# MiniMax-AI/VTP

Measured on AMD Instinct MI355X. Metric: images/sec/node VTP-B f16d64 256x256 train step, higher is better.
Workload: dtype bf16

## Files before the change

vtp_amd/csrc/gemm4w_tn.hip:

```cpp
#include "gemm_common.h"
#include "gemm_group.h"
#include "diag.h"
#include "gemm4w_tn_ktile.inc"

namespace vtp {

namespace {
constexpr int W4T_KT = 65536;
constexpr int W4T_RING = 2 * W4T_KT;
constexpr int W4T_LDS = W4T_RING + 32768;
}

__device__ __forceinline__ void w4t_glds16(const char* sbase, unsigned voff, unsigned lds_dst) {
  unsigned keep;
  asm volatile("s_mov_b32 %0, m0\n\ts_mov_b32 m0, %3\n\ts_nop 0\n\tglobal_load_lds_dwordx4 %1, %2\n\ts_mov_b32 m0, %0"
               : "=&s"(keep)
               : "v"(voff), "s"(sbase), "s"(lds_dst)
               : "memory");
}

__device__ __forceinline__ int w4t_uni(long v) { return __builtin_amdgcn_readfirstlane((int)v); }
template <class T>
__device__ __forceinline__ T* w4t_uni(T* v) {
  const unsigned long long u = (unsigned long long)v;
  const unsigned lo = __builtin_amdgcn_readfirstlane((unsigned)u), hi = __builtin_amdgcn_readfirstlane((unsigned)(u >> 32));
  return (T*)(((unsigned long long)hi << 32) | lo);
}

struct W4TStage {
  const char *mata, *matb, *zb;
  unsigned stepa, stepb, da[2], db[2];
};

__device__ __forceinline__ void w4t_kloop(bool csum, f32x16 (&acc)[4][4], float (&cs)[4], const unsigned (&aE)[2], const unsigned (&aO)[2],
                                          const unsigned (&bE)[2], const unsigned (&bO)[2], unsigned& pea, unsigned& peb, unsigned zoff,
                                          const W4TStage& st, int& kra, int& krb, unsigned nk2) {
  unsigned vt, sm, cnt = nk2;
  unsigned long long sb;
  const unsigned ones = 0x3F803F80u;
  const unsigned docs = __builtin_amdgcn_readfirstlane(csum ? 1u : 0u);
  asm volatile(W4T_TILE_ASM_BOTH
               : W4T_TILE_ACC, [cs0] "+v"(cs[0]), [cs1] "+v"(cs[1]), [cs2] "+v"(cs[2]), [cs3] "+v"(cs[3]), [pea] "+v"(pea), [peb] "+v"(peb),
                 [vt] "=&v"(vt), [kra] "+s"(kra), [krb] "+s"(krb), [cnt] "+s"(cnt), [sm] "=&s"(sm), [sb] "=&s"(sb)
               : [aE0] "v"(aE[0]), [aO0] "v"(aO[0]), [bE0] "v"(bE[0]), [bO0] "v"(bO[0]), [aE1] "v"(aE[1]), [aO1] "v"(aO[1]), [bE1] "v"(bE[1]),
                 [bO1] "v"(bO[1]), [zoff] "v"(zoff), [mata] "s"(st.mata), [matb] "s"(st.matb), [zb] "s"(st.zb), [stepa] "s"(st.stepa),
                 [stepb] "s"(st.stepb), [ones] "s"(ones), [docs] "s"(docs), [da0] "s"(st.da[0]), [da1] "s"(st.da[1]), [db0] "s"(st.db[0]),
                 [db1] "s"(st.db[1])
               : "memory", "scc", "vcc", W4T_TILE_CLOBBERS);
}

__device__ __forceinline__ void w4t_segment(const GroupArgs& ga, int tile, int kbeg, int kcount, int nparts, int part) {
  extern __shared__ __attribute__((aligned(16))) char smem[];
  const int tid = threadIdx.x;
  auto stamp = [&](int which) {
    if (__builtin_expect(ga.timing != nullptr, 0) && tid == 0) diag_stamp(ga.timing, (size_t)blockIdx.x * 8 + which);
  };
  if (__builtin_expect(ga.timing != nullptr, 0) && tid == 0) {
    ga.timing[(size_t)blockIdx.x * 8 + 5] = (unsigned long long)tile;
    ga.timing[(size_t)blockIdx.x * 8 + 6] = (unsigned long long)part;
    unsigned xcc;
    asm volatile("s_getreg_b32 %0, hwreg(HW_REG_XCC_ID)" : "=s"(xcc));
    ga.timing[(size_t)blockIdx.x * 8 + 7] = (unsigned long long)(xcc & 15);
  }
  stamp(0);
  const int lane = tid & 63;
  const int wave = __builtin_amdgcn_readfirstlane(tid >> 6);
  const int wr = wave >> 1, wc = wave & 1;
  const int hi = lane >> 5;

  int g = 0;
  for (int i = 1; i < ga.nprob; ++i)
    if ((int)ga.probs[i].tile0 <= tile) g = i;
  const GroupProblem& pr = ga.probs[g];
  GemmArgs p{};
  p.A = w4t_uni(pr.A); p.B = w4t_uni(pr.B); p.C = w4t_uni(pr.C); p.resid = w4t_uni(pr.accumulate) ? (const float*)p.C : nullptr;
  p.colsum = w4t_uni(pr.colsum);
  p.M = w4t_uni(pr.M); p.N = w4t_uni(pr.N); p.K = w4t_uni(pr.K) > 0 ? w4t_uni(pr.K) : ga.K; p.lda = w4t_uni(pr.lda); p.ldb = w4t_uni(pr.ldb); p.ldc = w4t_uni(pr.ldc);
  p.c_grp = w4t_uni(pr.c_grp); p.c_pre = w4t_uni(pr.c_pre); p.k_split = ga.k_split; p.alpha = 1.f;
  p.xcd_swizzle = 2;
  const int lt = tile - w4t_uni(pr.tile0), tiles_n = (p.N + 255) >> 8;
  const int n0 = (lt % tiles_n) << 8, m0 = (lt / tiles_n) << 8;
  kcount = max(0, min(kcount, p.K - kbeg));
  const unsigned nk2 = (unsigned)max(1, (kcount + 127) >> 7);

  const int krow = lane >> 3, chunk = (lane & 7) ^ (4 * ((krow >> 1) & 1));
  const int cola = min(m0 + wave * 64 + chunk * 8, p.M - 8), colb = min(n0 + wave * 64 + chunk * 8, p.N - 8);
  unsigned pea = (unsigned)(((size_t)(kbeg + krow) * p.lda + cola) * 2), peb = (unsigned)(((size_t)(kbeg + krow) * p.ldb + colb) * 2);
  const unsigned zoff = (lane & 3) * 16;
  W4TStage st;
  st.mata = (const char*)p.A;
  st.matb = (const char*)p.B;
  st.zb = (const char*)g_zero_block;
  st.stepa = (unsigned)(8 * p.lda * 2);
  st.stepb = (unsigned)(8 * p.ldb * 2);
#pragma unroll
  for (int sl = 0; sl < 2; ++sl) {
    st.da[sl] = (unsigned)(size_t)smem + sl * W4T_KT + wave * 8192;
    st.db[sl] = st.da[sl] + 32768;
  }
#pragma unroll
  for (int kt = 0; kt < 2; ++kt)
#pragma unroll
    for (int i = 0; i < 8; ++i) {
      const bool valid = kt * 64 + 8 * i < kcount;
      w4t_glds16(valid ? st.mata : st.zb, valid ? pea : zoff, st.da[kt] + i * 1024);
      w4t_glds16(valid ? st.matb : st.zb, valid ? peb : zoff, st.db[kt] + i * 1024);
      pea += st.stepa;
      peb += st.stepb;
    }
  int kra = kcount - 128, krb = kcount - 128;

  unsigned aE[2], aO[2], bE[2], bO[2];
  {
    const int t_li = lane & 15, t_rq = t_li >> 2;
    const int cq = ((lane >> 4) & 1) * 2 + ((t_li & 3) >> 1), sz = 4 * ((t_rq >> 1) & 1);
    const unsigned rowb = (unsigned)((hi * 8 + t_rq) * 128 + (t_li & 1) * 8);
    const unsigned lb0 = rowb + (unsigned)(((0 + cq) ^ sz) << 4), lb1 = rowb + (unsigned)(((4 + cq) ^ sz) << 4);
#pragma unroll
    for (int sl = 0; sl < 2; ++sl) {
      const unsigned ba = (unsigned)(size_t)smem + sl * W4T_KT + (wr * 2) * 8192, bb = (unsigned)(size_t)smem + sl * W4T_KT + (4 + wc * 2) * 8192;
      aE[sl] = ba + lb0;
      aO[sl] = ba + lb1;
      bE[sl] = bb + lb0;
      bO[sl] = bb + lb1;
    }
  }
  f32x16 acc[4][4];
#pragma unroll
  for (int i = 0; i < 4; ++i)
#pragma unroll
    for (int j = 0; j < 4; ++j)
#pragma unroll
      for (int e = 0; e < 16; ++e) acc[i][j][e] = 0.f;
  float cs[4] = {0.f, 0.f, 0.f, 0.f};
  const bool do_csum = p.colsum != nullptr && n0 == 0;

  asm volatile("s_waitcnt vmcnt(0)" ::: "memory");
  __builtin_amdgcn_s_barrier();
  __builtin_amdgcn_sched_barrier(0);
  stamp(1);
  w4t_kloop(do_csum, acc, cs, aE, aO, bE, bO, pea, peb, zoff, st, kra, krb, nk2);
  asm volatile("s_nop 15\n\ts_nop 15\n\ts_nop 7\n\ts_waitcnt vmcnt(0)" ::: "memory");
  stamp(2);

  if (do_csum && wc == 0) {
#pragma unroll
    for (int j = 0; j < 4; ++j) {
      const float v = cs[j] + __shfl_xor(cs[j], 32, 64);
      const int m = m0 + wr * 128 + j * 32 + (lane & 31);
      if (hi == 0 && m < p.M) unsafeAtomicAdd(p.colsum + remap_row(m, p.c_grp, p.c_pre), v);
    }
  }
  if (nparts > 1) {
    typedef __attribute__((ext_vector_type(4))) unsigned int u32x4_t;
    const f32x4* mine = (const f32x4*)ga.part + (((size_t)tile * ga.splits + part) * 4 + wave) * 4096;
    const auto rsrc = __builtin_amdgcn_make_buffer_rsrc((void*)mine, 0, 4096 * 16, 0x00020000);
#pragma unroll
    for (int u = 0; u < 64; ++u) {
      f32x4 v;
#pragma unroll
      for (int e = 0; e < 4; ++e) v[e] = acc[u >> 4][(u >> 2) & 3][4 * (u & 3) + e];
      __builtin_amdgcn_raw_buffer_store_b128((u32x4_t)v, rsrc, lane * 16 + u * 1024, 0,  16);
    }
    asm volatile("s_waitcnt vmcnt(0)" ::: "memory");
    __syncthreads();
    int* flag = (int*)(smem + W4T_LDS - 16);
    if (tid == 0) {
      const int t = __hip_atomic_fetch_add(ga.ticket + tile, 1, __ATOMIC_RELAXED, __HIP_MEMORY_SCOPE_AGENT);
      const int last = t == nparts - 1;
      if (last) {
        __builtin_amdgcn_fence(__ATOMIC_ACQUIRE, "agent");
        __hip_atomic_store(ga.ticket + tile, 0, __ATOMIC_RELAXED, __HIP_MEMORY_SCOPE_AGENT);
      }
      *flag = last;
    }
    __syncthreads();
    stamp(3);
    if (*flag == 0) return;
    for (int z = 0; z < nparts; ++z) {
      if (z == part) continue;
      const f32x4* other = (const f32x4*)ga.part + (((size_t)tile * ga.splits + z) * 4 + wave) * 4096 + lane;
      constexpr int NLD = 16;
#pragma unroll
      for (int gq = 0; gq < 64 / NLD; ++gq) {
        f32x4 v[NLD];
#pragma unroll
        for (int t = 0; t < NLD; ++t) v[t] = other[(gq * NLD + t) * 64];
#pragma unroll
        for (int t = 0; t < NLD; ++t) {
          const int u = gq * NLD + t;
#pragma unroll
          for (int e = 0; e < 4; ++e) acc[u >> 4][(u >> 2) & 3][4 * (u & 3) + e] += v[t][e];
        }
        asm volatile("" ::: "memory");
      }
    }
  }
  char* reg = smem + W4T_RING + wave * 8192;
  gemm_epilogue<EPI_F32, false, 128, 64, 4096, 0>(p, *(f32x16(*)[2][4]) & acc[0], reg, m0, n0, wr, wc * 2, lane, 0, nullptr);
  gemm_epilogue<EPI_F32, false, 128, 64, 4096, 0>(p, *(f32x16(*)[2][4]) & acc[2], reg, m0, n0, wr, wc * 2 + 1, lane, 0, nullptr);
  stamp(4);
}


__global__ __launch_bounds__(256, 1) void gemm4w_grouped_tn_items_kernel(const GroupArgs ga) {
  const int c = xcd_chunk_start(blockIdx.x, gridDim.x) + ((int)blockIdx.x >> 3);
  const GroupItem& it = ga.items[c];
  w4t_segment(ga, w4t_uni(it.tile), w4t_uni(it.kbeg), w4t_uni(it.kcount), w4t_uni(it.nparts), w4t_uni(it.part));
}

int launch_gemm4w_grouped_tn_items(const GroupArgs& ga, int nitems, hipStream_t s) {
  static bool attr_set = false;
  if (!attr_set) {
    (void)hipFuncSetAttribute((const void*)gemm4w_grouped_tn_items_kernel, hipFuncAttributeMaxDynamicSharedMemorySize, W4T_LDS);
    attr_set = true;
  }
  hipLaunchKernelGGL(gemm4w_grouped_tn_items_kernel, dim3(nitems), dim3(256), W4T_LDS, s, ga);
  return check_launch("gemm4w_grouped_tn_items");
}

}
```

vtp_amd/csrc/gemm8p.hip:

```cpp
#include "gemm_common.h"
#include "gemm_group.h"
#include "diag.h"
#include <cstdlib>
#include <type_traits>

namespace vtp {

namespace {
constexpr int P8_SLOT = 16384;
constexpr int P8_RING = 8 * P8_SLOT;
constexpr int P8_REGION = 4096;
constexpr int P8_LDS = P8_RING + 8 * P8_REGION;
}

__device__ __forceinline__ void p8_wait_vm_halftiles(int n) {
  if (n >= 4) asm volatile("s_waitcnt vmcnt(8)" ::: "memory");
  else if (n == 3) asm volatile("s_waitcnt vmcnt(6)" ::: "memory");
  else if (n == 2) asm volatile("s_waitcnt vmcnt(4)" ::: "memory");
  else if (n == 1) asm volatile("s_waitcnt vmcnt(2)" ::: "memory");
  else asm volatile("s_waitcnt vmcnt(0)" ::: "memory");
}

__device__ __forceinline__ void p8_glds16(const char* sbase, unsigned voff, unsigned lds_dst) {
  unsigned keep;
// ... 562 lines not shown
    return launch_persistent<kern, gemm8p_dyn_kernel<EPI, VAR, XMODE>>(a, ntiles, 1, 512, P8_LDS, 4, s, "gemm8p_nt");
  else
    return launch_persistent<kern, nullptr>(a, ntiles, 1, 512, P8_LDS, 4, s, TRANS ? "gemm8p_tn" : "gemm8p_nt");
}

bool gemm8p_fits(const GemmArgs& a, bool trans) {
  const size_t lim = (size_t)1 << 32;
  if (trans) return (size_t)a.K * a.lda * 2 < lim && (size_t)a.K * a.ldb * 2 < lim;
  size_t rows_a = a.M;
  if (a.a_grp > 0) rows_a += ((size_t)a.M / a.a_grp + 1) * a.a_pre;
  return rows_a * a.lda * 2 < lim && (size_t)a.N * a.ldb * 2 < lim;
}

int launch_gemm8p_nt(const GemmArgs& a, int epi, int splits, hipStream_t s) {
  switch (epi) {
    case EPI_BF16:
      if (a.rope_pos) return launch8p<EPI_BF16, false, 0, 1>(a, splits, s);
      if (a.swiglu_pre) return launch8p<EPI_BF16, false, 0, 2>(a, splits, s);
      return launch8p<EPI_BF16, false, 0, 0>(a, splits, s);
    case EPI_F32: return launch8p<EPI_F32, false>(a, splits, s);
    case EPI_SWIGLU: return launch8p<EPI_SWIGLU, false>(a, splits, s);
    case EPI_GELU: return launch8p<EPI_GELU, false>(a, splits, s);
    case EPI_F32_ATOMIC: return launch8p<EPI_F32_ATOMIC, false>(a, splits, s);
    case EPI_F32_SLAB: return launch8p<EPI_F32_SLAB, false>(a, splits, s);
    default: set_error("gemm8p: unsupported epilogue %d", epi); return VTP_ERR_ARG;
  }
}

int launch_gemm8p_nt_fp8(const GemmArgs& a, int epi, hipStream_t s) {
  switch (epi) {
    case EPI_BF16: return a.rope_pos ? launch8p<EPI_BF16, false, 8, 1>(a, 1, s) : launch8p<EPI_BF16, false, 8, 0>(a, 1, s);
    case EPI_F32: return launch8p<EPI_F32, false, 8>(a, 1, s);
    case EPI_SWIGLU: return launch8p<EPI_SWIGLU, false, 8>(a, 1, s);
    default: set_error("gemm8p fp8: unsupported epilogue %d", epi); return VTP_ERR_ARG;
  }
}

int launch_gemm8p_tn(const GemmArgs& a, int epi, int splits, hipStream_t s) {
  if (epi == EPI_F32) return launch8p<EPI_F32, true>(a, 1, s);
  if (epi == EPI_F32_ATOMIC) return launch8p<EPI_F32_ATOMIC, true>(a, splits, s);
  return launch8p<EPI_F32_SLAB, true>(a, splits, s);
}

}

namespace vtp {
int launch_gemm4w_grouped_tn_items(const GroupArgs& ga, int nitems, hipStream_t s);
}
static int launch_gemm8p_grouped_tn(const void* probs, int nprob, int ntiles, int K, int splits, void* part, void* ticket,
                                    const int* k_rows, void* stream) {
  using namespace vtp;
  if (k_rows) { splits = 1; part = ticket = nullptr; }
  GroupArgs ga{};
  ga.probs = (const GroupProblem*)probs; ga.part = (float*)part; ga.ticket = (int*)ticket;
  ga.nprob = nprob; ga.ntiles = ntiles; ga.K = K;
  ga.k_split = ((K + splits - 1) / splits + 63) / 64 * 64;
  ga.splits = (K + ga.k_split - 1) / ga.k_split;
  ga.timing = g_p8_timing;
  ga.k_rows = k_rows;
  auto* kern = k_rows ? gemm8p_grouped_tn_limit_kernel : gemm8p_grouped_tn_kernel;
  static bool attr_set[2] = {false, false};
  if (!attr_set[k_rows != nullptr]) {
    hipFuncSetAttribute((const void*)kern, hipFuncAttributeMaxDynamicSharedMemorySize, P8_LDS);
    attr_set[k_rows != nullptr] = true;
  }
  hipLaunchKernelGGL(kern, dim3(ntiles * ga.splits), dim3(512), P8_LDS, (hipStream_t)stream, ga);
  return check_launch("gemm8p_grouped_tn");
}
extern "C" int vtp_gemm_tn_grouped(const void* probs, int nprob, int ntiles, int K, int splits, void* part, void* ticket,
                                   void* stream) {
  VTP_REQUIRE(probs && nprob >= 1 && nprob <= 8, "vtp_gemm_tn_grouped: 1..8 problems");
  VTP_REQUIRE(ntiles >= 1 && K >= 1 && splits >= 1, "vtp_gemm_tn_grouped: bad shape (ntiles %d, K %d, splits %d)", ntiles, K, splits);
  VTP_REQUIRE(splits == 1 || (part && ticket), "vtp_gemm_tn_grouped: split-K needs the partial-sum and ticket buffers");
  return launch_gemm8p_grouped_tn(probs, nprob, ntiles, K, splits, part, ticket, nullptr, stream);
}
extern "C" int vtp_gemm_tn_grouped_limit(const void* probs, int nprob, int ntiles, int K, const int* k_rows, void* stream) {
  VTP_REQUIRE(probs && k_rows && nprob >= 1 && nprob <= 8, "vtp_gemm_tn_grouped_limit: 1..8 problems and a row count");
  VTP_REQUIRE(ntiles >= 1 && K >= 1, "vtp_gemm_tn_grouped_limit: bad shape (ntiles %d, K %d)", ntiles, K);
  return launch_gemm8p_grouped_tn(probs, nprob, ntiles, K, 1, nullptr, nullptr, k_rows, stream);
}
extern "C" int vtp_gemm_tn_grouped_items(const void* probs, int nprob, int ntiles, int K, const void* items, int nitems, int slots,
                                         void* part, void* ticket, void* stream) {
  using namespace vtp;
  VTP_REQUIRE(probs && nprob >= 1 && nprob <= 8, "vtp_gemm_tn_grouped_items: 1..8 problems");
  VTP_REQUIRE(items && nitems >= ntiles && ntiles >= 1 && K >= 8 && K % 8 == 0 && slots >= 1,
              "vtp_gemm_tn_grouped_items: bad shape (ntiles %d, nitems %d, K %d, slots %d)", ntiles, nitems, K, slots);
  VTP_REQUIRE(slots == 1 || (part && ticket), "vtp_gemm_tn_grouped_items: split tiles need the partial-sum and ticket buffers");
  GroupArgs ga{};
  ga.probs = (const GroupProblem*)probs; ga.part = (float*)part; ga.ticket = (int*)ticket;
  ga.nprob = nprob; ga.ntiles = ntiles; ga.K = K; ga.k_split = K; ga.splits = slots;
  ga.timing = g_p8_timing;
  ga.items = (const GroupItem*)items;
  return launch_gemm4w_grouped_tn_items(ga, nitems, (hipStream_t)stream);
}

extern "C" int vtp_set_gemm_dynamic(int on) {
  vtp::g_dyn_mode = on ? 1 : 0;
  return VTP_OK;
}

extern "C" int vtp_gemm_debug(void* timing, int grid_limit, int delay_ticks) {
  const bool off = timing == nullptr && grid_limit == 0 && delay_ticks == 0;
  if (!off && !vtp::diag_allowed("vtp_gemm_debug")) return VTP_ERR_ARG;
  if (delay_ticks < 0 || grid_limit < 0) {
    vtp::set_error("vtp_gemm_debug: negative grid limit / delay");
    return VTP_ERR_ARG;
  }
  vtp::g_p8_timing = (unsigned long long*)timing;
  vtp::g_p8_grid = grid_limit;
  vtp::g_p8_delay = delay_ticks;
  return VTP_OK;
}
```

vtp_amd/engine.py:

```python
from __future__ import annotations

import math
import os
from typing import Dict, List, NamedTuple, Optional, Tuple

import torch

from . import ops
from .ops import EPI_BF16, EPI_F32, EPI_F32_SLAB, EPI_GELU, EPI_SWIGLU


class Lin:
    __slots__ = ("N", "K", "w", "wT", "bias", "gw", "gb", "w32", "wTs")


class SwiGLULin:
    __slots__ = ("H", "K", "w12", "w12T", "b12", "gw1", "gb1")


def _flat_order(names: List[str]) -> List[str]:
    out, seen = [], set()
    for n in names:
        if n in seen:
            continue
# ... 767 lines not shown
        xmid = ws.get("xmid", (M, D), F32)
        hid = ws.get("hid", (M, H), BF)
        rope_plan = self._rope_plan(ws, segs, prefix_tokens, M)
        rope_arg = None if rope_plan is None else (rope_plan[0], rope_plan[1], rope_plan[2], 2 * D)
        rows = self._attn_rows(segs)
        for i, b in enumerate(self.blocks):
            w8, al, sc = f["w"][i], f["alpha"][i], f["act_scale"][i]
            xout = ws.get(f"xout{i & 1}", (M, D), F32)
            ops.norm_fwd_e4m3(x, b.n1w, b.n1b, a8, sc[0:1], None, M, D, self.eps, self.kind)
            if b.qn_w is not None:
                qkv_pre = ws.get("f8.qkv_pre", (M, 3 * D), BF)
                ops.gemm_nt_fp8(a8, w8[0], qkv_pre, M=M, N=3 * D, K=D, alpha=al[0], bias=b.qkv.bias, epi=EPI_BF16)
                ops.qk_norm_fwd(qkv_pre, b.qn_w, b.kn_w, qkv, ws.get("f8.qinv", (M, 2 * heads), F32), M, D)
            else:
                ops.gemm_nt_fp8(a8, w8[0], qkv, M=M, N=3 * D, K=D, alpha=al[0], bias=b.qkv.bias, epi=EPI_BF16, rope=rope_arg)
            self._attention(qkv, o, lse, rows, i, prefix_tokens, rope_arg is None)
            ops.quantize_e4m3(o, a8, sc[1:2])
            ops.gemm_nt_fp8(a8, w8[1], xmid, M=M, N=D, K=D, alpha=al[1], bias=b.proj.bias, resid=x, epi=EPI_F32)
            ops.norm_fwd_e4m3(xmid, b.n2w, b.n2b, a8, sc[2:3], None, M, D, self.eps, self.kind)
            ops.gemm_nt_fp8(a8, w8[2], hid, M=M, N=2 * H, K=D, alpha=al[2], bias=b.w12.b12, epi=EPI_SWIGLU)
            ops.quantize_e4m3(hid, a8, sc[3:4])
            ops.gemm_nt_fp8(a8, w8[3], xout, M=M, N=D, K=H, alpha=al[3], bias=b.w3.bias, resid=xmid, epi=EPI_F32)
            x = xout
        return x

    def fp32_check(self, what: str):
        if self.qk_norm:
            raise NotImplementedError(f"fp32 forward ({what}): QK normalisation (use_qk_norm) is not implemented in fp32")
        if self.D % 8 or self.H % 8 or self.D != self.heads * 64:
            raise NotImplementedError(f"fp32 forward ({what}): needs D, H multiples of 8 and head dimension 64 (D={self.D} H={self.H} heads={self.heads})")

    def _forward_fp32(self, ws: Workspace, x, segs, prefix_tokens: int, M: int, keep: bool = False):
        self.fp32_check(self.style)
        D, H, heads = self.D, self.H, self.heads
        xn, st = ws.get("f32.xn", (M, D), F32), ws.get("f32.st", (M, 2), F32)
        qkv, o = ws.get("f32.qkv", (M, 3 * D), F32), ws.get("f32.o", (M, D), F32)
        xmid, hid = ws.get("f32.xmid", (M, D), F32), ws.get("f32.hid", (M, H), F32)
        rows = self._attn_rows(segs)
        for i, b in enumerate(self.blocks):
            xout = ws.get(f"f32.{i}.xout" if keep else f"f32.xout{i & 1}", (M, D), F32)
            ops.norm_fwd_f32(x, b.n1w, b.n1b, xn, st, M, D, self.eps, self.kind)
            ops.gemm_nt_f32(xn, b.qkv.w32, qkv, M=M, N=3 * D, K=D, bias=b.qkv.bias)
            for r0, Bs, Ns, rp in rows:
                q_s, o_s = qkv[r0:r0 + Bs * Ns], o[r0:r0 + Bs * Ns]
                if rp is not None:
                    rs, rc = rope_at(rp, i)
                    ops.rope_qk_f32(q_s, rs, rc, Bs, Ns, heads, prefix_tokens)
                ops.attn_fwd_f32(q_s, q_s[:, D:], q_s[:, 2 * D:], o_s, Bs, Ns, heads, Ns * 3 * D, 3 * D, Ns * D, D, ATTN_SCALE, self.causal)
            ops.gemm_nt_f32(o, b.proj.w32, xmid, M=M, N=D, K=D, bias=b.proj.bias, gamma=b.ls1, resid=x, epi=ops.F32_RESID)
            ops.norm_fwd_f32(xmid, b.n2w, b.n2b, xn, st, M, D, self.eps, self.kind)
            if self.swiglu:
                ops.gemm_nt_f32(xn, b.w1_32, hid, M=M, N=H, K=D, w2=b.w2_32, bias=b.b1_32, bias2=b.b2_32, epi=ops.F32_SWIGLU)
            else:
                ops.gemm_nt_f32(xn, b.fc.w32, hid, M=M, N=H, K=D, bias=b.fc.bias,
                                epi=ops.F32_QUICK_GELU if self.quick_gelu else ops.F32_GELU)
            ops.gemm_nt_f32(hid, b.w3.w32, xout, M=M, N=D, K=H, bias=b.w3.bias, gamma=b.ls2, resid=xmid, epi=ops.F32_RESID)
            x = xout
        return x

    def w3_colsum_target(self, i: int):
        b = self.blocks[i]
        return b.w3.gb if (b.ls2 is None and self.drop_plan is None) else None

    def backward(self, ws: Workspace, dy, dy_b, segs, prefix_tokens: int, saved=None, dy_colsum_done: bool = False,
                 hold_last: bool = False, extra_last=None):
        D, H = self.D, self.H
        M = sum(b * n for b, n, _ in segs)
        saved = self.last_saved if saved is None else saved
        tail_Mc = saved[-1].o_c.shape[0] if saved and saved[-1].row_map is not None else None
        drop = self.drop_plan is not None
        if drop:
            csegs, Mb = self._drop_segs(segs)
            rows, scales, bt = list(self._rows(csegs)), self.drop_plan["scales"], "b.d."
            gdy, gdy_b = ws.get(bt + "gdy", (Mb, D), F32), ws.get(bt + "gdy_b", (Mb, D), BF)
            dxc = ws.get(bt + "dxc", (Mb, D), F32)
        else:
            Mb, rows, bt = M, self._attn_rows(segs), "b."
            dmid = ws.get("b.dmid", (M, D), F32)
        grouped = not drop and M >= 256 and all(b.ls1 is None and b.ls2 is None for b in self.blocks) \
            and ops.wgrad_group_fits(M, max(3 * D, 2 * H if self.swiglu else H)) and D % 8 == 0 and H % 8 == 0
        vl = self.varlen
        if vl is not None and not (grouped and tail_Mc is None and len(segs) == 1 and not extra_last):
            raise RuntimeError("Stack.backward: packed captions need the grouped weight gradients of one plain segment (varlen_ok)")
        par = (lambda i: f".{i & 1}") if grouped else (lambda i: "")
        groups = ws.__dict__.setdefault("_wgrad_groups", {})
        scratch = self.__dict__.setdefault("_wgrad_scratch", {})
        pending = None

        def launch_pending():
            if pending is None:
                return
            if OVERLAP.enabled:
                OVERLAP.fork()
                side, grp = OVERLAP.side, pending[1]

                def issue():
                    with torch.cuda.stream(side):
                        grp.launch()
                OVERLAP.defer(issue)
            else:
                pending[1].launch()

        for i in range(self.depth - 1, -1, -1):
            b, s = self.blocks[i], saved[i]
            t = f"{i}.d." if drop else f"{i}."
            dpre = ws.get(bt + "dx12" + par(i), (Mb, 2 * H if self.swiglu else H), BF)
            dqkv = ws.get(bt + "dqkv" + par(i), (Mb, 3 * D), BF)
            if drop:
                self._gather(dy, segs, csegs, i, 1, gdy, gdy_b, scales)
                self._ffn_bwd(ws, i, s, gdy, gdy_b, dxc, None, Mb, bt, dpre, fused=False)
                self._scatter(dxc, dy, segs, csegs, i, 1, 1.0, accumulate=False)
                self._gather(dy, segs, csegs, i, 0, gdy, gdy_b, scales)
                self._attn_bwd(ws, t, i, s, gdy, gdy_b, dxc, None, Mb, bt, dqkv, rows, prefix_tokens)
                self._scatter(dxc, dy, segs, csegs, i, 0, 1.0, accumulate=False)
                OVERLAP.join()
                yield ("block", i)
                continue
            dxo = ws.get(f"b.dx{i & 1}", (M, D), F32)
            dxo_b = ws.get(f"b.dx_b{i & 1}", (M, D), BF)
            Mf = tail_Mc if (tail_Mc is not None and i == self.depth - 1) else M
            if Mf != M:
                dpre = ws.get(bt + "dx12" + par(i), (Mf, 2 * H if self.swiglu else H), BF)
            dmid = ws.get("b.dmid", (Mf, D), F32)
            dmid_b = ws.get("b.dmid_b" + par(i), (Mf, D), BF)
            probs = [] if grouped else None
            if grouped:
                launch_pending()
            self._ffn_bwd(ws, i, s, dy, dy_b, dmid, dmid_b, Mf, bt, dpre, fused=self.swiglu and b.ls2 is None,
                          bias_done=dy_colsum_done if i == self.depth - 1 else self.w3_colsum_target(i) is not None, probs=probs,
                          dx_colsum=b.proj.gb if b.ls1 is None else None)
            self._attn_bwd(ws, t, i, s, dmid, dmid_b, dxo, dxo_b, M, bt, dqkv, rows, prefix_tokens, bias_done=b.proj.gb is not None,
                           probs=probs, join=grouped, dx_colsum=self.w3_colsum_target(i - 1) if i > 0 else None)
            dy, dy_b = dxo, dxo_b
            if not grouped:
                OVERLAP.join()
                yield ("block", i)
                continue
            extra = [dict(pr, dy=dy_b) for pr in extra_last] if (i == 0 and hold_last and extra_last) else []
            gkey = (i, bool(self.wgrad_overwrite), len(extra), Mf, vl is not None)
            grp = groups.get(gkey)
            if grp is None:
                counts = sorted({pr.get("Ktok", M) for pr in probs + extra}, reverse=True)
                if len(counts) > 1 and ops.wgrad_group_mixed_ok(counts):
                    counts = [None]
                parts = []
                for kt in counts:
                    g = ops.WgradGroup(M if kt is None else kt, k_rows=self.m_rows)
                    for pr in probs + extra:
                        if kt is None or pr.get("Ktok", M) == kt:
                            g.add(pr["dy"], pr["x"], pr["gw"], pr["gb"], pr["N"], pr["K"], pr["swiglu_h"],
                                  accumulate=not self.wgrad_overwrite, Ktok=pr.get("Ktok"))
                    parts.append(g.finalize(self.store.device, scratch))
                grp = groups[gkey] = parts[0] if len(parts) == 1 else WgradGroups(parts)
            if pending is not None:
                yield ("block", pending[0])
            pending = (i, grp)
        self.held = None
        if drop:
            ops.cast_f32_bf16(dy, dy_b, M * D)
        elif pending is not None and hold_last:
            OVERLAP.run_deferred()
            self.held = pending
        elif pending is not None:
            pending[1].launch()
            yield ("block", pending[0])
        return dy, dy_b


_ROPE_CACHE: Dict[tuple, Tuple[torch.Tensor, torch.Tensor]] = {}


def _rope_host(per: torch.Tensor, H: int, W: int, aug=None) -> Tuple[torch.Tensor, torch.Tensor]:
    dd = {"dtype": per.dtype}
    ch = torch.arange(0.5, H, **dd) / H
    cw = torch.arange(0.5, W, **dd) / W
    coords = torch.stack(torch.meshgrid(ch, cw, indexing="ij"), dim=-1).flatten(0, 1)
    coords = 2.0 * coords - 1.0
    if aug is not None:
        if aug.get("shift") is not None:
            coords += aug["shift"][None, :]
        if aug.get("jitter") is not None:
            coords *= aug["jitter"][None, :]
        if aug.get("rescale") is not None:
            coords *= aug["rescale"]
    ang = 2 * math.pi * coords[:, :, None] / per[None, None, :]
    ang = ang.flatten(1, 2).tile(2)
    return torch.sin(ang).to(torch.bfloat16).contiguous(), torch.cos(ang).to(torch.bfloat16).contiguous()


def rope_tables(periods: torch.Tensor, H: int, W: int, device) -> Tuple[torch.Tensor, torch.Tensor]:
    per = periods.detach().to("cpu")
    key = (H, W, str(device), per.dtype, tuple(per.float().tolist()))
    hit = _ROPE_CACHE.get(key)
    if hit is not None:
        return hit
    sin, cos = _rope_host(per, H, W)
    sin, cos = sin.to(device), cos.to(device)
    _ROPE_CACHE[key] = (sin, cos)
    return sin, cos


class RopeAugTabs:
    __slots__ = ("sin_all", "cos_all", "off", "hw")

    def __init__(self, sin_all, cos_all, off, hw):
        self.sin_all, self.cos_all, self.off, self.hw = sin_all, cos_all, off, hw

    def at(self, i: int):
        i = min(i, self.sin_all.shape[0] - 1)
        return self.sin_all[i, self.off:self.off + self.hw], self.cos_all[i, self.off:self.off + self.hw]


def rope_at(rp, i: int):
    return rp.at(i) if isinstance(rp, RopeAugTabs) else rp


def _rope_hw(rp) -> int:
    return rp.hw if isinstance(rp, RopeAugTabs) else rp[0].shape[0]


class RopeAugmenter:

    def __init__(self, periods: torch.Tensor, depth: int, per_block: bool, shift, jitter, rescale, seed: int = 0):
        self.per, self.depth, self.per_block = periods.detach().to("cpu"), depth, per_block
        self.cfg = (shift, jitter, rescale)
        self.engine_id = int(seed)
        self.gen = torch.Generator().manual_seed(int(seed))
        self.records: Dict[tuple, dict] = {}
        self.touched = set()
        self.last_draws = None

    def reseed(self, base_seed: int, rank: int = 0):
        self.gen.manual_seed((int(base_seed) * 1000003 + int(rank)) * 8 + self.engine_id)

    def get_state(self) -> torch.Tensor:
        return self.gen.get_state().clone()

    def set_state(self, state: torch.Tensor):
        self.gen.set_state(state.to("cpu", torch.uint8))

    @property
    def active(self) -> bool:
        return any(v is not None for v in self.cfg)

    def _draw(self):
        import numpy as np
        shift, jitter, rescale = self.cfg
        dd = {"dtype": self.per.dtype}
# ... 342 lines not shown
```

vtp_amd/ops.py:

```python
from __future__ import annotations

import torch

from . import _lib

EPI_BF16, EPI_F32, EPI_SWIGLU, EPI_GELU, EPI_F32_ATOMIC, EPI_F32_SLAB = 0, 1, 2, 3, 4, 5
EPI_QUICK_GELU = 8
NORM_RMS, NORM_LN = 0, 1


def _s():
    return torch.cuda.current_stream().cuda_stream


def _p(t):
    return 0 if t is None else t.data_ptr()


def _lib_():
    return _lib.load()


def pad8(n: int) -> int:
    return (n + 7) // 8 * 8
# ... 190 lines not shown
        v = int(os.environ.get("VTP_GEMM_CUS", "0") or 0)
    except ValueError:
        v = 0
    return v - v % 8 if 8 <= v < 256 else 256


def wgrad_group_splits(ntiles: int, Ktok: int):
    s = max(1, min(gemm_cus() // ntiles, Ktok // 1024))
    ks = ((Ktok + s - 1) // s + 63) // 64 * 64
    return ks, (Ktok + ks - 1) // ks


def wgrad_group_kernel(ntiles: int, splits: int, Ktok: int) -> int:
    import os
    e = os.environ.get("VTP_GEMM4W_TN")
    if Ktok % 8 != 0 or e == "0":
        return 0
    if e == "1":
        return 1
    return 1 if Ktok // max(splits, 1) >= W4_TN_MIN_SLICE else 0


def wgrad_k_cuts(Ktok: int, n: int):
    ks = ((Ktok + n - 1) // n + 63) // 64 * 64
    return [(b, min(Ktok, b + ks) - b) for b in range(0, Ktok, ks)]


def wgrad_group_items(rows, Ktok: int, base_splits: int, cus: int = None):
    cus = gemm_cus() if cus is None else cus
    tiles = []
    for pi, r in enumerate(rows):
        gb, N, K, tile0 = r[3], r[7], r[8], r[11]
        tn = (K + 255) // 256
        for lt in range(((N + 255) // 256) * tn):
            tiles.append((tile0 + lt, pi, gb != 0 and lt % tn == 0))
    ncs = sum(1 for t in tiles if t[2])
    Ks = [int(r[13]) or int(Ktok) for r in rows]
    if len(set(Ks)) > 1:
        per = wgrad_mixed_splits([sum(1 for t in tiles if t[1] == pi) for pi in range(len(rows))], Ks, cus)
    else:
        per = [base_splits] * len(rows)
    n_items = sum(per[t[1]] for t in tiles)
    items, slots = [], 1
    for pi in range(len(rows)):
        more = ncs > 0 and n_items + ncs <= cus and Ks[pi] // (per[pi] + 1) >= 1024
        for heavy in (True, False):
            grp = [t for t in tiles if t[1] == pi and t[2] == heavy]
            if not grp:
                continue
            cs = wgrad_k_cuts(Ks[pi], per[pi] + 1 if (heavy and more) else per[pi])
            slots = max(slots, len(cs))
            for z, (kb, kc) in enumerate(cs):
                items += [[t[0], kb, kc, len(cs), z, 0, 0, 0] for t in grp]
    return items, slots


def wgrad_mixed_splits(ntiles, Ks, cus: int):
    n = len(Ks)
    per = [1] * n
    length = lambda p: ((Ks[p] + per[p] - 1) // per[p] + 63) // 64 * 64
    while True:
        top = max(length(p) for p in range(n))
        grp = [p for p in range(n) if length(p) == top]
        total = sum(per[p] * ntiles[p] for p in range(n))
        if total + sum(ntiles[p] for p in grp) > cus or any(Ks[p] // (per[p] + 1) < 1024 for p in grp):
            return per
        for p in grp:
            per[p] += 1


def wgrad_group_mixed_ok(Ks) -> bool:
    import os
    e = os.environ.get("VTP_GEMM4W_TN")
    if e == "0" or any(k % 8 for k in Ks):
        return False
    return e == "1" or min(Ks) >= W4_TN_MIN_SLICE


def wgrad_group_uniform_items(ntiles: int, Ktok: int, splits: int):
    cs = wgrad_k_cuts(Ktok, max(int(splits), 1))
    return [[t, kb, kc, len(cs), z, 0, 0, 0] for z, (kb, kc) in enumerate(cs) for t in range(ntiles)], len(cs)


W4_TN_MIN_SLICE = 4096


class WgradGroup:

    def __init__(self, Ktok: int, k_rows=None):
        self.k_rows = k_rows
        self.Ktok, self.rows, self.ntiles, self.keep = int(Ktok), [], 0, []
        self.table = self.part = self.ticket = None
        self._uniform = {}

    def add(self, dy, x, gw, gb, N: int, K: int, swiglu_h: int = 0, accumulate: bool = True, Ktok: int = None):
        if N % 8 or K % 8 or dy.stride(0) % 8 or x.stride(0) % 8 or N < 8 or K < 8:
            raise ValueError(f"WgradGroup.add: N = {N}, K = {K} and the leading dimensions ({dy.stride(0)}, {x.stride(0)}) must be multiples "
                             "of 8 (use the per-layer weight-gradient path: linear_bwd without `defer`)")
        self.rows.append([dy.data_ptr(), x.data_ptr(), gw.data_ptr(), 0 if gb is None else gb.data_ptr(), dy.stride(0), x.stride(0), K,
                          N, K, -1 if swiglu_h else 0, swiglu_h, self.ntiles, int(accumulate), 0 if Ktok is None or int(Ktok) == self.Ktok else int(Ktok),
                          0, 0])
        self.ntiles += ((N + 255) // 256) * ((K + 255) // 256)
        self.keep += [dy, x, gw, gb]

    def finalize(self, device, scratch=None):
        import torch
        assert 1 <= len(self.rows) <= 8
        Ks = [r[13] or self.Ktok for r in self.rows]
        self.mixed = len(set(Ks)) > 1
        if not self.mixed and Ks[0] != self.Ktok:
            self.Ktok = Ks[0]
            for r in self.rows:
                r[13] = 0
        if self.mixed and any(k % 8 or k < 8 for k in Ks):
            raise ValueError(f"WgradGroup: problems over different token counts {Ks} need multiples of 8 (the item-list kernel); "
                             "launch one group per token count")
        if not all(wgrad_group_fits(k, max(r[4], r[5])) for k, r in zip(Ks, self.rows)):
            raise ValueError("WgradGroup: token rows x leading dimension exceed the 32-bit staging offsets of vtp_gemm_tn_grouped; "
                             "use the per-layer weight-gradient path (linear_bwd without `defer`)")
        _, self.splits = wgrad_group_splits(self.ntiles, self.Ktok)
        self.table = torch.tensor(self.rows, dtype=torch.int64, device=device)
        if self.k_rows is not None:
            if self.mixed:
                raise ValueError("WgradGroup: a device token count takes one static token count for every problem")
            self.splits, self.kernel, self.items, self.nitems, self.slots = 1, 0, None, None, 1
            return self
        self.kernel = 1 if self.mixed else wgrad_group_kernel(self.ntiles, self.splits, self.Ktok)
        self.items, self.nitems, self.slots = None, None, self.splits
        if self.kernel == 1:
            items, self.slots = wgrad_group_items(self.rows, self.Ktok, self.splits)
            self.nitems = len(items)
            self.items = torch.tensor(items, dtype=torch.int32, device=device)
        if self.slots > 1:
            scratch = {} if scratch is None else scratch
            need = self.ntiles * self.slots * 65536
            if scratch.get("part") is None or scratch["part"].numel() < need:
                scratch["part"] = torch.empty(need, dtype=torch.float32, device=device)
            if scratch.get("ticket") is None or scratch["ticket"].numel() < self.ntiles:
                scratch["ticket"] = torch.zeros(max(self.ntiles, 256), dtype=torch.int32, device=device)
            self.part, self.ticket = scratch["part"], scratch["ticket"]
        return self

    def launch(self, kernel=None):
        if kernel is None:
            kernel = self.kernel
        if self.k_rows is not None:
            if kernel != 0:
                raise ValueError("WgradGroup.launch: a device token count runs on the 8-phase kernel only")
            _lib.check(_lib_().vtp_gemm_tn_grouped_limit(_p(self.table), len(self.rows), self.ntiles, self.Ktok, _p(self.k_rows), _s()),
                       "vtp_gemm_tn_grouped_limit")
            return
        if kernel == 0 and self.mixed:
            raise ValueError("WgradGroup.launch: the 8-phase kernel takes one token count for every problem")
        if kernel == 0:
            _lib.check(_lib_().vtp_gemm_tn_grouped(_p(self.table), len(self.rows), self.ntiles, self.Ktok, self.splits, _p(self.part),
                                                   _p(self.ticket), _s()), "vtp_gemm_tn_grouped")
            return
        if kernel != 1:
            raise ValueError(f"WgradGroup.launch: kernel must be 0, 1 or None, not {kernel!r}")
        items, nitems, slots = self.items, self.nitems, self.slots
        if items is None:
            if self.splits not in self._uniform:
                import torch
                rows, slots = wgrad_group_uniform_items(self.ntiles, self.Ktok, self.splits)
                self._uniform[self.splits] = (torch.tensor(rows, dtype=torch.int32, device=self.table.device), len(rows), slots)
            items, nitems, slots = self._uniform[self.splits]
        _lib.check(_lib_().vtp_gemm_tn_grouped_items(_p(self.table), len(self.rows), self.ntiles, self.Ktok, _p(items), nitems, slots,
                                                     _p(self.part), _p(self.ticket), _s()), "vtp_gemm_tn_grouped_items")


def colsum_bf16(inp, ld, out, R, C, swiglu_h=0, in_remap=(0, 0)):
    _lib.check(_lib_().vtp_colsum_bf16(_p(inp), ld, _p(out), swiglu_h, in_remap[0], in_remap[1], R, C, _s()), "vtp_colsum_bf16")


def colsum_bf16_rows(inp, ld, out, n_rows_dev, R_max, C):
    _lib.check(_lib_().vtp_colsum_bf16_rows(_p(inp), ld, _p(out), _p(n_rows_dev), R_max, C, _s()), "vtp_colsum_bf16_rows")


def gather_image_rows(src, idx, dst, dst_bf16, n_img, N, D, scale=1.0):
    _lib.check(_lib_().vtp_gather_image_rows(_p(src), _p(idx), _p(dst), _p(dst_bf16), n_img, N, D, scale, _s()), "vtp_gather_image_rows")


def scatter_image_rows(src, idx, dst, n_img, N, D, alpha=1.0, accumulate=True):
    _lib.check(_lib_().vtp_scatter_image_rows(_p(src), _p(idx), _p(dst), n_img, N, D, alpha, int(accumulate), _s()),
               "vtp_scatter_image_rows")


def gather_tail_rows(o, x, idx, o_c, x_c, T, L, M, D):
    _lib.check(_lib_().vtp_gather_tail_rows(_p(o), _p(x), _p(idx), _p(o_c), _p(x_c), T, L, M, D, _s()), "vtp_gather_tail_rows")


def tail_row_map(idx, row_map, T, L, M):
    _lib.check(_lib_().vtp_tail_row_map(_p(idx), _p(row_map), T, L, M, _s()), "vtp_tail_row_map")


def expand_rows_bf16(src, row_map, dst, M, Mc, D):
    _lib.check(_lib_().vtp_expand_rows_bf16(_p(src), _p(row_map), _p(dst), M, Mc, D, _s()), "vtp_expand_rows_bf16")


def layerscale_wgrad(G, W, bias, colsum, gamma, dW, db, dgamma, N, K):
    _lib.check(_lib_().vtp_layerscale_wgrad(_p(G), _p(W), _p(bias), _p(colsum), _p(gamma), _p(dW), _p(db), _p(dgamma), N, K, _s()),
               "vtp_layerscale_wgrad")


def scaled_transpose(W, gamma, dstT, N, K):
    _lib.check(_lib_().vtp_scaled_transpose(_p(W), _p(gamma), _p(dstT), N, K, _s()), "vtp_scaled_transpose")


def gemm_splits(K, splits):
    return _lib_().vtp_gemm_splits(K, splits)


def gemm_tn_splits(M, N, K):
    return _lib_().vtp_gemm_tn_splits(M, N, K)


def reduce_slabs(slabs, stride, S, dst, n, accumulate=True):
    _lib.check(_lib_().vtp_reduce_slabs(_p(slabs), stride, S, _p(dst), n, int(accumulate), _s()), "vtp_reduce_slabs")


def ema(t, s, n, momentum):
    _lib.check(_lib_().vtp_ema(_p(t), _p(s), n, momentum, _s()), "vtp_ema")


def embed_tokens(ids, table, pos, x, eot, B, T, D):
    _lib.check(_lib_().vtp_embed_tokens(_p(ids), _p(table), _p(pos), _p(x), _p(eot), B, T, D, _s()), "vtp_embed_tokens")


def embed_tokens_bwd(ids, dx, d_table, d_pos, B, T, D):
    _lib.check(_lib_().vtp_embed_tokens_bwd(_p(ids), _p(dx), _p(d_table), _p(d_pos), B, T, D, _s()), "vtp_embed_tokens_bwd")


def gather_rows(x, idx, out, B, T, D):
    _lib.check(_lib_().vtp_gather_rows(_p(x), _p(idx), _p(out), B, T, D, _s()), "vtp_gather_rows")


# ... 752 lines not shown
```

Measured before the change: 765.8.

## Pair weight-gradient groups of two blocks into one grouped GEMM launch

In the backward stack, alternate blocks now defer their weight-gradient problems and merge them with the next block's problems into one grouped GEMM of up to 16 problems. This is gated on the combined tile count fitting in the CU count. It cuts the number of wgrad launches and fills more CUs per launch, and uses a three-way buffer rotation for the bf16 dx and intermediates so the deferred block's inputs stay live. The item kernel also gets a SPLIT template parameter so unsplit launches compile out the partial-sum reduction path. The cost is extra workspace and a delayed gradient finish for the carried block.

```diff
diff --git a/vtp_amd/csrc/gemm4w_tn.hip b/vtp_amd/csrc/gemm4w_tn.hip
--- a/vtp_amd/csrc/gemm4w_tn.hip
+++ b/vtp_amd/csrc/gemm4w_tn.hip
@@ -49,6 +49,7 @@
                : "memory", "scc", "vcc", W4T_TILE_CLOBBERS);
 }
 
+template <bool SPLIT>
 __device__ __forceinline__ void w4t_segment(const GroupArgs& ga, int tile, int kbeg, int kcount, int nparts, int part) {
   extern __shared__ __attribute__((aligned(16))) char smem[];
   const int tid = threadIdx.x;
@@ -151,7 +152,7 @@
       if (hi == 0 && m < p.M) unsafeAtomicAdd(p.colsum + remap_row(m, p.c_grp, p.c_pre), v);
     }
   }
-  if (nparts > 1) {
+  if (SPLIT && nparts > 1) {
     typedef __attribute__((ext_vector_type(4))) unsigned int u32x4_t;
     const f32x4* mine = (const f32x4*)ga.part + (((size_t)tile * ga.splits + part) * 4 + wave) * 4096;
     const auto rsrc = __builtin_amdgcn_make_buffer_rsrc((void*)mine, 0, 4096 * 16, 0x00020000);
@@ -203,20 +204,26 @@
 }
 
 
+template <bool SPLIT>
 __global__ __launch_bounds__(256, 1) void gemm4w_grouped_tn_items_kernel(const GroupArgs ga) {
   const int c = xcd_chunk_start(blockIdx.x, gridDim.x) + ((int)blockIdx.x >> 3);
   const GroupItem& it = ga.items[c];
-  w4t_segment(ga, w4t_uni(it.tile), w4t_uni(it.kbeg), w4t_uni(it.kcount), w4t_uni(it.nparts), w4t_uni(it.part));
-}
-
-int launch_gemm4w_grouped_tn_items(const GroupArgs& ga, int nitems, hipStream_t s) {
+  w4t_segment<SPLIT>(ga, w4t_uni(it.tile), w4t_uni(it.kbeg), w4t_uni(it.kcount), SPLIT ? w4t_uni(it.nparts) : 1, w4t_uni(it.part));
+}
+
+template <bool SPLIT>
+static int launch_w4t_items(const GroupArgs& ga, int nitems, hipStream_t s) {
   static bool attr_set = false;
   if (!attr_set) {
-    (void)hipFuncSetAttribute((const void*)gemm4w_grouped_tn_items_kernel, hipFuncAttributeMaxDynamicSharedMemorySize, W4T_LDS);
+    (void)hipFuncSetAttribute((const void*)gemm4w_grouped_tn_items_kernel<SPLIT>, hipFuncAttributeMaxDynamicSharedMemorySize, W4T_LDS);
     attr_set = true;
   }
-  hipLaunchKernelGGL(gemm4w_grouped_tn_items_kernel, dim3(nitems), dim3(256), W4T_LDS, s, ga);
+  hipLaunchKernelGGL(gemm4w_grouped_tn_items_kernel<SPLIT>, dim3(nitems), dim3(256), W4T_LDS, s, ga);
   return check_launch("gemm4w_grouped_tn_items");
 }
 
-}
+int launch_gemm4w_grouped_tn_items(const GroupArgs& ga, int nitems, hipStream_t s) {
+  return ga.splits > 1 ? launch_w4t_items<true>(ga, nitems, s) : launch_w4t_items<false>(ga, nitems, s);
+}
+
+}
diff --git a/vtp_amd/csrc/gemm8p.hip b/vtp_amd/csrc/gemm8p.hip
--- a/vtp_amd/csrc/gemm8p.hip
+++ b/vtp_amd/csrc/gemm8p.hip
@@ -668,7 +668,7 @@
 extern "C" int vtp_gemm_tn_grouped_items(const void* probs, int nprob, int ntiles, int K, const void* items, int nitems, int slots,
                                          void* part, void* ticket, void* stream) {
   using namespace vtp;
-  VTP_REQUIRE(probs && nprob >= 1 && nprob <= 8, "vtp_gemm_tn_grouped_items: 1..8 problems");
+  VTP_REQUIRE(probs && nprob >= 1 && nprob <= 16, "vtp_gemm_tn_grouped_items: 1..16 problems");
   VTP_REQUIRE(items && nitems >= ntiles && ntiles >= 1 && K >= 8 && K % 8 == 0 && slots >= 1,
               "vtp_gemm_tn_grouped_items: bad shape (ntiles %d, nitems %d, K %d, slots %d)", ntiles, nitems, K, slots);
   VTP_REQUIRE(slots == 1 || (part && ticket), "vtp_gemm_tn_grouped_items: split tiles need the partial-sum and ticket buffers");
diff --git a/vtp_amd/engine.py b/vtp_amd/engine.py
--- a/vtp_amd/engine.py
+++ b/vtp_amd/engine.py
@@ -873,7 +873,13 @@
         vl = self.varlen
         if vl is not None and not (grouped and tail_Mc is None and len(segs) == 1 and not extra_last):
             raise RuntimeError("Stack.backward: packed captions need the grouped weight gradients of one plain segment (varlen_ok)")
-        par = (lambda i: f".{i & 1}") if grouped else (lambda i: "")
+        tiles = lambda N, K: ((N + 255) // 256) * ((K + 255) // 256)
+        paired = grouped and vl is None and self.depth >= 4 and ops.wgrad_pair_ok(
+            2 * (tiles(3 * D, D) + tiles(D, D) + tiles(2 * H if self.swiglu else H, D) + tiles(D, H)), M)
+        upper = (lambda i: i <= self.depth - 2 and i >= 2 and (self.depth - 2 - i) % 2 == 0) if paired else (lambda i: False)
+        gen = (lambda i: f"{i % 3}") if paired else (lambda i: f"{i & 1}")
+        par = (lambda i: "." + gen(i)) if grouped else (lambda i: "")
+        carry = None
         groups = ws.__dict__.setdefault("_wgrad_groups", {})
         scratch = self.__dict__.setdefault("_wgrad_scratch", {})
         pending = None
@@ -908,7 +914,7 @@
                 yield ("block", i)
                 continue
             dxo = ws.get(f"b.dx{i & 1}", (M, D), F32)
-            dxo_b = ws.get(f"b.dx_b{i & 1}", (M, D), BF)
+            dxo_b = ws.get("b.dx_b" + gen(i), (M, D), BF)
             Mf = tail_Mc if (tail_Mc is not None and i == self.depth - 1) else M
             if Mf != M:
                 dpre = ws.get(bt + "dx12" + par(i), (Mf, 2 * H if self.swiglu else H), BF)
@@ -928,7 +934,16 @@
                 yield ("block", i)
                 continue
             extra = [dict(pr, dy=dy_b) for pr in extra_last] if (i == 0 and hold_last and extra_last) else []
-            gkey = (i, bool(self.wgrad_overwrite), len(extra), Mf, vl is not None)
+            if upper(i):
+                if pending is not None:
+                    for j in pending[0]:
+                        yield ("block", j)
+                pending, carry = None, (i, probs)
+                continue
+            blocks_of = (i,)
+            if carry is not None:
+                blocks_of, probs, carry = (carry[0], i), carry[1] + probs, None
+            gkey = (blocks_of if paired else i, bool(self.wgrad_overwrite), len(extra), Mf, vl is not None)
             grp = groups.get(gkey)
             if grp is None:
                 counts = sorted({pr.get("Ktok", M) for pr in probs + extra}, reverse=True)
@@ -944,17 +959,18 @@
                     parts.append(g.finalize(self.store.device, scratch))
                 grp = groups[gkey] = parts[0] if len(parts) == 1 else WgradGroups(parts)
             if pending is not None:
-                yield ("block", pending[0])
-            pending = (i, grp)
+                for j in pending[0]:
+                    yield ("block", j)
+            pending = (blocks_of, grp)
         self.held = None
         if drop:
             ops.cast_f32_bf16(dy, dy_b, M * D)
         elif pending is not None and hold_last:
             OVERLAP.run_deferred()
-            self.held = pending
+            self.held = (pending[0][0], pending[1])
         elif pending is not None:
             pending[1].launch()
-            yield ("block", pending[0])
+            yield ("block", pending[0][0])
         return dy, dy_b
 
 
diff --git a/vtp_amd/ops.py b/vtp_amd/ops.py
--- a/vtp_amd/ops.py
+++ b/vtp_amd/ops.py
@@ -296,6 +296,14 @@
     return [[t, kb, kc, len(cs), z, 0, 0, 0] for z, (kb, kc) in enumerate(cs) for t in range(ntiles)], len(cs)
 
 
+def wgrad_pair_ok(ntiles: int, Ktok: int) -> bool:
+    import os
+    if os.environ.get("VTP_WGRAD_PAIR", "1") in ("0", "false", "off"):
+        return False
+    return ntiles <= gemm_cus() and Ktok <= W4_TN_PAIR_MAX_ROWS and wgrad_group_kernel(ntiles, 1, Ktok) == 1
+
+
+W4_TN_PAIR_MAX_ROWS = 12288
 W4_TN_MIN_SLICE = 4096
 
 
@@ -319,7 +327,7 @@
 
     def finalize(self, device, scratch=None):
         import torch
-        assert 1 <= len(self.rows) <= 8
+        assert 1 <= len(self.rows) <= 16
         Ks = [r[13] or self.Ktok for r in self.rows]
         self.mixed = len(set(Ks)) > 1
         if not self.mixed and Ks[0] != self.Ktok:
@@ -332,6 +340,9 @@
         if not all(wgrad_group_fits(k, max(r[4], r[5])) for k, r in zip(Ks, self.rows)):
             raise ValueError("WgradGroup: token rows x leading dimension exceed the 32-bit staging offsets of vtp_gemm_tn_grouped; "
                              "use the per-layer weight-gradient path (linear_bwd without `defer`)")
+        if len(self.rows) > 8 and (self.k_rows is not None or any(k % 8 or k < 8 for k in Ks)):
+            raise ValueError("WgradGroup: more than 8 problems run on the item-list kernel only (token counts multiples of 8, no device "
+                             "token count)")
         _, self.splits = wgrad_group_splits(self.ntiles, self.Ktok)
         self.table = torch.tensor(self.rows, dtype=torch.int64, device=device)
         if self.k_rows is not None:
@@ -339,7 +350,7 @@
                 raise ValueError("WgradGroup: a device token count takes one static token count for every problem")
             self.splits, self.kernel, self.items, self.nitems, self.slots = 1, 0, None, None, 1
             return self
-        self.kernel = 1 if self.mixed else wgrad_group_kernel(self.ntiles, self.splits, self.Ktok)
+        self.kernel = 1 if self.mixed or len(self.rows) > 8 else wgrad_group_kernel(self.ntiles, self.splits, self.Ktok)
         self.items, self.nitems, self.slots = None, None, self.splits
         if self.kernel == 1:
             items, self.slots = wgrad_group_items(self.rows, self.Ktok, self.splits)
@@ -366,6 +377,8 @@
             return
         if kernel == 0 and self.mixed:
             raise ValueError("WgradGroup.launch: the 8-phase kernel takes one token count for every problem")
+        if kernel == 0 and len(self.rows) > 8:
+            raise ValueError("WgradGroup.launch: the 8-phase kernel takes at most 8 problems")
         if kernel == 0:
             _lib.check(_lib_().vtp_gemm_tn_grouped(_p(self.table), len(self.rows), self.ntiles, self.Ktok, self.splits, _p(self.part),
                                                    _p(self.ticket), _s()), "vtp_gemm_tn_grouped")
```

Measured after the change: 768.4, median of 2. No clear change (+0.3%).
